# EnricoMiccoli/nodal

Hardware: AMD Instinct MI355X
Metric: circuits_per_sec (higher is better)
Workload: dtype f64; 1 GPU; cfg3: grid(1000) 1e6 nodes, sparse CSR path; n=999999, nnz=4995995, parallelism=one GPU

## Files before the change

nodal_amd/csrc/sagg.hip:

```cpp
#include <hip/hip_ext.h>

#include <atomic>
#include <type_traits>

#include "group.h"

int grounded_flags(nodal_ctx *h, uint8_t *flags_dev);

namespace {

using grp::TB;
constexpr int PW = 4;
constexpr int ACAP = 64;
constexpr int RCAP = 96;
constexpr int RCAP_SMALL = 512;
constexpr int RCAP_SMALL_ROWS = 16384;
inline int rcap_for(int64_t nc) { return nc <= RCAP_SMALL_ROWS ? RCAP_SMALL : RCAP; }
constexpr int W0_MAX = 32;
constexpr int COARSEST = 64;
constexpr int MAX_LEVELS = 12;
constexpr int MIS_ROUNDS = 6;
constexpr int TAIL_MAX_N = 1024;
constexpr int TAIL_LEVELS = 6;
constexpr int TAIL_LDS_BUDGET = 150 * 1024;
// ... 94 lines not shown
    bool kcycle = true;
    bool kfrozen = false;
    int kslot = -1, kcount = 0, ksamples = 0;
    int klevels = 1;
    int nu[3] = {2, 1, 2};
    bool dense_coarsest = true;
    DevBuf tail_stamps, tail_image, apcol, apval, aplen, bstat;
    DevBuf tail_op;
    bool tail_dense = false;
    DevBuf mvec;
    hipEvent_t ev_copy = nullptr;
    hipStream_t aux = nullptr;
    hipEvent_t ev_fork = nullptr, ev_join = nullptr, ev_flags = nullptr;
    bool aux_pending = false;
    bool aux_tried = false;
    bool want_flags = false;
    int flags_levels = 0;
    DevBuf stats, coarse_inv, mis_t, mis_m, mis_flag, mis_id, agg1, keys, rstart, cursor, lists;
    TailDesc td;
    uint64_t *host_stats = nullptr;
    bool sym_valid = false;
    uint64_t sym_epoch = 0;
    int64_t sym_n = 0, sym_nnz = 0;
    bool sym_general = false, sym_check = false;
    int32_t sym_floating = 0;
    hipGraph_t it_graph = nullptr;
    hipGraphExec_t it_exec = nullptr;
    uint64_t it_key = 0;
    bool refreshed = false;
    int last_iters = 0;
    int hint_iters = 0;
    int64_t hint_n = 0, hint_nnz = 0;
    int mblock_iters = 0;
    int64_t mblock_n = 0;
    unsigned long long sym_stats[MAX_LEVELS * ST_COUNT] = {0};
    SLevel *level(int l) {
        while ((int)pool.size() <= l) pool.push_back(new SLevel());
        return pool[l];
    }
    void drop_graph() {
        if (it_exec) (void)hipGraphExecDestroy(it_exec);
        if (it_graph) (void)hipGraphDestroy(it_graph);
        it_exec = nullptr;
        it_graph = nullptr;
        it_key = 0;
    }
    ~SHierarchy() {
        drop_graph();
        if (ev_copy) (void)hipEventDestroy(ev_copy);
        if (ev_fork) (void)hipEventDestroy(ev_fork);
        if (ev_join) (void)hipEventDestroy(ev_join);
        if (ev_flags) (void)hipEventDestroy(ev_flags);
        if (aux) (void)hipStreamDestroy(aux);
        for (SLevel *l : pool) {
            DevBuf *b[] = {&l->acol, &l->aval, &l->alen, &l->dinv, &l->agg, &l->pcol, &l->pval, &l->rcol,
                           &l->rval, &l->rlen, &l->vec, &l->part, &l->gflag, &l->avalf, &l->pvalf, &l->rvalf, &l->adcol,
                           &l->wcol, &l->wval, &l->wlen};
            for (DevBuf *x : b) x->release();
            delete l;
        }
        tail_image.release();
        tail_op.release();
        mvec.release();
        tail_stamps.release();
        bstat.release();
        apcol.release();
        apval.release();
        aplen.release();
        DevBuf *b[] = {&stats, &coarse_inv, &mis_t, &mis_m, &mis_flag, &mis_id, &agg1, &keys, &rstart, &cursor, &lists};
        for (DevBuf *x : b) x->release();
        if (host_stats) (void)hipHostFree(host_stats);
    }
};


constexpr int BSTAT_MAX = 65536;
__global__ __launch_bounds__(1024) void reduce_bstat(int nblocks, const uint32_t *__restrict__ bstat,
                                                     unsigned long long *__restrict__ stats, int slot_max,
                                                     int slot_sum) {
    __shared__ unsigned int s_max;
    __shared__ unsigned long long s_sum;
    if (threadIdx.x == 0) { s_max = 0; s_sum = 0; }
    __syncthreads();
    unsigned int m = 0;
    unsigned long long t = 0;
    for (int i = threadIdx.x; i < nblocks; i += 1024) {
        m = max(m, bstat[i]);
        t += bstat[BSTAT_MAX + i];
// ... 41 lines not shown
    if (far) atomicOr(&s_bad, 2u);
    __syncthreads();
    if (threadIdx.x == 0) {
        bstat[blockIdx.x] = s_len;
        bstat[BSTAT_MAX + blockIdx.x] = s_graded;
        if (s_bad & 1u) atomicOr(&stats[ST_BADDIAG], 1ull);
        if (s_bad & 2u) stats[ST_FARCOL] = 1ull;
    }
}

__global__ __launch_bounds__(TB) void csr_to_ell(int64_t n, int64_t ld, const int32_t *__restrict__ indptr,
                                                 const int32_t *__restrict__ indices,
                                                 const double *__restrict__ data, int32_t *__restrict__ col,
                                                 double *__restrict__ val, float *__restrict__ valf,
                                                 int32_t *__restrict__ len, double *__restrict__ dinv, int32_t wpad,
                                                 int16_t *__restrict__ dcol) {
    for (int64_t i = (int64_t)xcd_block() * TB + threadIdx.x; i < n; i += (int64_t)gridDim.x * TB) {
        const int32_t e0 = indptr[i], e1 = indptr[i + 1];
        double d = 1.0;
        for (int32_t e = e0; e < e1; ++e) {
            const int32_t c = indices[e];
            const double v = data[e];
            col[(int64_t)(e - e0) * ld + i] = c;
            if (dcol) dcol[(int64_t)(e - e0) * ld + i] = (int16_t)(c - (int32_t)i);
            val[(int64_t)(e - e0) * ld + i] = v;
            valf[(int64_t)(e - e0) * ld + i] = (float)v;
            if (c == (int32_t)i) d = v;
        }
        for (int32_t s = e1 - e0; s < wpad; ++s) {
            col[(int64_t)s * ld + i] = (int32_t)i;
            if (dcol) dcol[(int64_t)s * ld + i] = 0;
            val[(int64_t)s * ld + i] = 0.0;
            valf[(int64_t)s * ld + i] = 0.0f;
        }
        len[i] = e1 - e0;
// ... 1200 lines not shown
    for (int i = 0; i < n; ++i) {
        long double y = 0.0L, a = 0.0L;
        for (int j = 0; j < n; ++j) {
            y += (long double)T[(size_t)i * n + j] * b[j];
            a += fabsl((long double)T[(size_t)i * n + j] * b[j]);
        }
        const double den = (double)a;
        const double q = fabs(yd[i] - yc[i]) / den, qp = (double)(fabsl((long double)yd[i] - y) / a);
        d = !(q <= d) ? q : d;
        dp = !(qp <= dp) ? qp : dp;
    }
    fprintf(stderr, "[sagg] tail check: n_t %d, dense operator against the cycle d = %.3e (product alone %.3e)\n", n, d, dp);
    return NODAL_OK;
}

int form_tail_op(nodal_ctx *h, SHierarchy *H) {
    static const bool on = !(getenv("NODAL_SA_TAIL_DENSE") && atoi(getenv("NODAL_SA_TAIL_DENSE")) == 0);
    H->tail_dense = false;
    if (!on || H->tail < 0) return NODAL_OK;
    const TailDesc &d = H->td;
    const int n = d.lv[0].n;
    static std::atomic<int> cus[64];
    const int dev = h->device >= 0 && h->device < 64 ? h->device : 0;
    int ncu = cus[dev].load(std::memory_order_acquire);
    if (ncu == 0) {
        NODAL_HIP_TRY(h, hipDeviceGetAttribute(&ncu, hipDeviceAttributeMultiprocessorCount, h->device >= 0 ? h->device : 0));
        if (ncu < 1) ncu = 1;
        cus[dev].store(ncu, std::memory_order_release);
    }
    NODAL_HIP_TRY(h, H->tail_op.reserve((size_t)n * n * 8 + 64));
    const unsigned gr = (unsigned)(n < ncu ? n : ncu);
    double *T = H->tail_op.as<double>();
    const char *img = H->tail_image.as<char>();
    if (d.slots <= 8) k_tail_pack_op<8><<<gr, 1024, (size_t)d.lds_bytes, h->stream>>>(d, img, T);
// ... 68 lines not shown
                    "(worst row against its own bound: %.3e)\n", l, (long long)n, (int)L->wslots, (int)L->maxlen, dm, qm);
    return NODAL_OK;
}
int fold_self_check(nodal_ctx *h, SHierarchy *H) {
    static const bool check = getenv("NODAL_TRACE") && getenv("NODAL_SA_FOLD_CHECK") && atoi(getenv("NODAL_SA_FOLD_CHECK")) != 0;
    if (!check) return NODAL_OK;
    for (int l = 0; l + 1 < H->nlev; ++l) {
        if (!H->pool[l]->fold) continue;
        const bool last = l + 1 == H->tail || l + 1 == H->nlev - 1;
        if (last) NODAL_TRY(fold_check_level<double>(h, H, l, false));
        else NODAL_TRY(fold_check_level<cyc_t>(h, H, l, true));
    }
    return NODAL_OK;
}

int build_tail(nodal_ctx *h, SHierarchy *H, const unsigned long long *hs) {
    H->tail = -1;
    H->tail_dense = false;
    const int last = H->nlev - 1;
    auto up16 = [](int x) { return (x + 15) & ~15; };
    for (int t = 1; t <= last; ++t) {
        if (H->pool[t]->n > TAIL_MAX_N || last - t + 1 > TAIL_LEVELS) continue;
        TailDesc d;
        memset(&d, 0, sizeof d);
        d.nlev = last - t + 1;
        d.nu = getenv("NODAL_SA_TAIL_NU") ? atoi(getenv("NODAL_SA_TAIL_NU")) : 3;
        if (d.nu < 1) d.nu = 1;
        int off = 0;
        for (int k = 0; k < d.nlev; ++k) {
            const SLevel *L = H->pool[t + k];
// ... 39 lines not shown
        d.slots = d.nlev > 1 ? (d.lv[0].width + d.lv[0].lpr - 1) / d.lv[0].lpr : 1;
        if (d.slots > 32) continue;
        {
            static std::atomic<bool> lds_allowed[64][3];
            const int dev = h->device >= 0 && h->device < 64 ? h->device : 0;
            const int which = d.slots <= 8 ? 0 : (d.slots <= 16 ? 1 : 2);
            if (!lds_allowed[dev][which].load(std::memory_order_acquire)) {
                NODAL_HIP_TRY(h, hipFuncSetAttribute(tail_kernel(d.slots), hipFuncAttributeMaxDynamicSharedMemorySize,
                                                     TAIL_LDS_BUDGET));
                NODAL_HIP_TRY(h, hipFuncSetAttribute(tail_op_kernel(d.slots), hipFuncAttributeMaxDynamicSharedMemorySize,
                                                     TAIL_LDS_BUDGET));
                lds_allowed[dev][which].store(true, std::memory_order_release);
            }
        }
        NODAL_HIP_TRY(h, H->tail_image.reserve((size_t)d.image_bytes + 256));
        k_tail_pack<<<1, 1024, 0, h->stream>>>(d, H->tail_image.as<char>());
        NODAL_HIP_TRY(h, hipGetLastError());
        H->td = d;
        H->tail = t;
        NODAL_TRY(form_tail_op(h, H));
        break;
    }
    return NODAL_OK;
}

int sagg_refresh(nodal_ctx *h, SHierarchy *H, const int32_t *indptr0, const int32_t *indices0, const double *data0,
                 bool general, bool *ok) {
    *ok = false;
    hipStream_t st = h->stream;
    unsigned long long *dstats = H->stats.as<unsigned long long>();
    unsigned long long *hs = reinterpret_cast<unsigned long long *>(H->host_stats);
    NODAL_HIP_TRY(h, hipMemsetAsync(dstats, 0, (size_t)MAX_LEVELS * ST_COUNT * 8, st));
    SLevel *L0 = H->pool[0];
    const int64_t n0 = L0->n;
    {
        const unsigned gr = grid_for(n0);
        static const double spread = getenv("NODAL_SA_SPREAD") ? atof(getenv("NODAL_SA_SPREAD")) : 16.0;
        static const double share = getenv("NODAL_SA_SHARE") ? atof(getenv("NODAL_SA_SHARE")) : 0.9;
        row_stats<<<gr, TB, 0, st>>>(n0, indptr0, indices0, data0, share, spread, general, dstats, H->bstat.as<uint32_t>());
        reduce_bstat<<<1, 1024, 0, st>>>((int)gr, H->bstat.as<uint32_t>(), dstats, ST_MAXLEN, ST_GRADED);
    }
    csr_to_ell<<<grid_for(n0), TB, 0, st>>>(n0, L0->ld, indptr0, indices0, data0, L0->acol.as<int32_t>(),
                                           L0->aval.as<double>(), L0->avalf.as<float>(),
                                           L0->alen.as<int32_t>(), L0->dinv.as<double>(), L0->wfix,
                                           L0->d16 ? L0->adcol.as<int16_t>() : nullptr);
    NODAL_HIP_TRY(h, hipGetLastError());
    for (int l = 0; l + 1 < H->nlev; ++l) {
        SLevel *L = H->pool[l], *C = H->pool[l + 1];
        Ell A = L->A();
        A.width = L->maxlen;
        build_P<<<grid_for(L->n), TB, 0, st>>>(A, L->dinv.as<double>(), L->agg.as<int32_t>(), L->pcol.as<int32_t>(),
                                              L->pval.as<double>(), L->pvalf.as<float>(), omega_p(l));
        const bool forked = H->aux != nullptr && nodal_extra_streams_ok(h) &&
                            !(getenv("NODAL_SA_FORK") && atoi(getenv("NODAL_SA_FORK")) == 0);
        hipStream_t rst = st;
        if (forked) {
            NODAL_HIP_TRY(h, hipEventRecord(H->ev_fork, st));
            NODAL_HIP_TRY(h, hipStreamWaitEvent(H->aux, H->ev_fork, 0));
            H->aux_pending = true;
            NODAL_TRY(galerkin_product<true>(h, H, l, nullptr, 1));
// ... 21 lines not shown
        if (hs[(size_t)k * ST_COUNT + ST_BADDIAG] || hs[(size_t)k * ST_COUNT + ST_OVERFLOW]) return NODAL_OK;
    decide_folds(H, hs, false);
    NODAL_TRY(fold_self_check(h, H));
    *ok = true;
    return NODAL_OK;
}

}

void sagg_destroy(nodal_ctx *h) {
    delete static_cast<SHierarchy *>(h->sagg);
    h->sagg = nullptr;
}

static int sagg_setup_csr_body(nodal_ctx *h, int64_t n0, int64_t nnz0, const int32_t *indptr0, const int32_t *indices0,
                               const double *data0, bool general, bool check_floating, bool *accepted, int32_t *floating);

int sagg_setup_csr(nodal_ctx *h, int64_t n0, int64_t nnz0, const int32_t *indptr0, const int32_t *indices0,
                   const double *data0, bool general, bool check_floating, bool *accepted, int32_t *floating) {
    const int s = sagg_setup_csr_body(h, n0, nnz0, indptr0, indices0, data0, general, check_floating, accepted, floating);
    SHierarchy *H = static_cast<SHierarchy *>(h->sagg);
    if (H && H->aux && H->aux_pending && H->ev_flags) {
        if (hipEventRecord(H->ev_flags, H->aux) == hipSuccess) (void)hipStreamWaitEvent(h->stream, H->ev_flags, 0);
        H->aux_pending = false;
        (void)hipGetLastError();
    }
    return s;
}

static int sagg_setup_csr_body(nodal_ctx *h, int64_t n0, int64_t nnz0, const int32_t *indptr0, const int32_t *indices0,
                               const double *data0, bool general, bool check_floating, bool *accepted, int32_t *floating) {
    *accepted = false;
    *floating = 0;
    static const bool enabled = !(getenv("NODAL_SAGG") && atoi(getenv("NODAL_SAGG")) == 0);
    static const bool trace = getenv("NODAL_TRACE") != nullptr;
    if (!enabled) return NODAL_OK;
    SHierarchy *H = hierarchy_of(h);
    H->ready = false;
    hipStream_t st = h->stream;
    if (n0 >= (1ll << 30)) return NODAL_OK;
    static const bool reuse = !(getenv("NODAL_SA_REUSE") && atoi(getenv("NODAL_SA_REUSE")) == 0);
    if (reuse && H->sym_valid && H->sym_epoch == h->struct_epoch && H->sym_n == n0 && H->sym_nnz == nnz0 &&
        H->sym_general == general && H->sym_check == check_floating) {
        bool ok = false;
        NODAL_TRY(sagg_refresh(h, H, indptr0, indices0, data0, general, &ok));
        if (ok) {
            *floating = H->sym_floating;
            H->refreshed = true;
            H->ready = true;
            *accepted = true;
            if (trace) fprintf(stderr, "[sagg] symbolic setup kept (struct epoch %llu): values refreshed\n",
                               (unsigned long long)h->struct_epoch);
            return NODAL_OK;
        }
        if (trace) fprintf(stderr, "[sagg] the kept hierarchy does not take the new values: full setup\n");
    }
    H->sym_valid = false;
    H->refreshed = false;
    H->want_flags = check_floating;
    H->flags_levels = 0;
    H->last_iters = 0;
    H->drop_graph();
    NODAL_HIP_TRY(h, H->stats.reserve((size_t)MAX_LEVELS * ST_COUNT * 8 + 64));
    if (!H->host_stats)
        NODAL_HIP_TRY(h, hipHostMalloc(reinterpret_cast<void **>(&H->host_stats), (size_t)MAX_LEVELS * ST_COUNT * 8 + 64));
    unsigned long long *dstats = H->stats.as<unsigned long long>();
    unsigned long long *hs = reinterpret_cast<unsigned long long *>(H->host_stats);
    NODAL_HIP_TRY(h, hipMemsetAsync(dstats, 0, (size_t)MAX_LEVELS * ST_COUNT * 8, st));
    NODAL_HIP_TRY(h, H->bstat.reserve((size_t)2 * BSTAT_MAX * 4 + 64));
    {
        const unsigned gr = grid_for(n0);
        static const double spread = getenv("NODAL_SA_SPREAD") ? atof(getenv("NODAL_SA_SPREAD")) : 16.0;
        static const double share = getenv("NODAL_SA_SHARE") ? atof(getenv("NODAL_SA_SHARE")) : 0.9;
        row_stats<<<gr, TB, 0, st>>>(n0, indptr0, indices0, data0, share, spread, general, dstats, H->bstat.as<uint32_t>());
        reduce_bstat<<<1, 1024, 0, st>>>((int)gr, H->bstat.as<uint32_t>(), dstats, ST_MAXLEN, ST_GRADED);
    }
    NODAL_HIP_TRY(h, hipGetLastError());
    NODAL_HIP_TRY(h, hipMemcpyAsync(hs, dstats, ST_COUNT * 8, hipMemcpyDeviceToHost, st));
    NODAL_WAIT_STREAM(h, st);
    const int64_t bar = n0 / 100 < 32 ? (n0 / 100 > 0 ? n0 / 100 : 1) : 32;
    if (hs[ST_MAXLEN] > (unsigned long long)W0_MAX || hs[ST_MAXLEN] == 0 || hs[ST_BADDIAG] ||
        (int64_t)hs[ST_GRADED] >= bar) {
        if (trace)
            fprintf(stderr, "[sagg] declined: longest row %llu, graded nodes %llu (bar %lld), M-matrix %s\n",
                    hs[ST_MAXLEN], hs[ST_GRADED], (long long)bar, hs[ST_BADDIAG] ? "no" : "yes");
        return NODAL_OK;
    }
    SLevel *L0 = H->level(0);
    L0->n = n0;
    L0->ld = pad64(n0);
    L0->maxlen = (int32_t)hs[ST_MAXLEN];
    L0->nnz = nnz0;
    L0->wfix = choose_wfix(L0->maxlen, n0, nnz0, 8);
    L0->width = L0->wfix ? L0->wfix : L0->maxlen;
    NODAL_HIP_TRY(h, L0->acol.reserve((size_t)L0->width * L0->ld * 4 + 64));
    NODAL_HIP_TRY(h, L0->aval.reserve((size_t)L0->width * L0->ld * 8 + 64));
    NODAL_HIP_TRY(h, L0->avalf.reserve((size_t)L0->width * L0->ld * 4 + 64));
    NODAL_HIP_TRY(h, L0->alen.reserve((size_t)L0->ld * 4 + 64));
    NODAL_HIP_TRY(h, L0->dinv.reserve((size_t)L0->ld * 8 + 64));
    static const bool d16_env = !(getenv("NODAL_SA_D16") && atoi(getenv("NODAL_SA_D16")) == 0);
    L0->d16 = d16_env && hs[ST_FARCOL] == 0;
    if (L0->d16) NODAL_HIP_TRY(h, L0->adcol.reserve((size_t)L0->width * L0->ld * 2 + 64));
    csr_to_ell<<<grid_for(n0), TB, 0, st>>>(n0, L0->ld, indptr0, indices0, data0, L0->acol.as<int32_t>(),
                                           L0->aval.as<double>(), L0->avalf.as<float>(),
                                           L0->alen.as<int32_t>(), L0->dinv.as<double>(), L0->wfix,
                                           L0->d16 ? L0->adcol.as<int16_t>() : nullptr);
    NODAL_HIP_TRY(h, hipGetLastError());

    int l = 0;
    bool diag_last = false;
    for (;; ++l) {
        SLevel *L = H->level(l);
        if (L->n <= COARSEST && l > 0) break;
        if (l + 1 >= MAX_LEVELS) {
            if (trace) fprintf(stderr, "[sagg] declined: more than %d levels\n", MAX_LEVELS);
            return NODAL_OK;
        }
        bool declined = false, stop = false;
        NODAL_TRY(build_level(h, H, l, hs, &declined, &stop));
        if (declined) {
            if (trace)
                fprintf(stderr, "[sagg] declined at level %d (%lld rows): does not coarsen / over a cap / not positive "
// ... 39 lines not shown
        if (k > 0) {
            H->pool[k]->maxlen = (int32_t)s[ST_MAXLEN];
            H->pool[k]->nnz = (int64_t)s[ST_NNZ];
            H->pool[k]->wfix = choose_wfix(H->pool[k]->maxlen, H->pool[k]->n, H->pool[k]->nnz, APAD);
        }
        if (s[ST_OVERFLOW] || (k > 0 && s[ST_BADDIAG]) || s[ST_UNASSIGNED]) {
            if (trace) fprintf(stderr, "[sagg] declined: level %d over a cap / not positive\n", k);
            return NODAL_OK;
        }
    }
    diag_last = last->maxlen <= 1;
    H->dense_coarsest = !diag_last;
    if (H->dense_coarsest) {
        if (last->n > COARSEST) return NODAL_OK;
        NODAL_HIP_TRY(h, H->coarse_inv.reserve((size_t)last->n * last->n * 8 + 64));
        coarsest_inverse<<<1, 256, 0, st>>>(last->A(), H->coarse_inv.as<double>(),
                                            dstats + (size_t)l * ST_COUNT);
        NODAL_HIP_TRY(h, hipGetLastError());
    }
    for (int k = 0; k < H->nlev; ++k) {
        SLevel *L = H->pool[k];
        NODAL_HIP_TRY(h, L->vec.reserve((size_t)V_COUNT * L->ld * 8 + 256));
        NODAL_HIP_TRY(h, L->part.reserve(5 * DOT_BLOCKS * 8 + 512));
    }
    NODAL_TRY(build_tail(h, H, hs));

    if (!check_floating) {
        NODAL_HIP_TRY(h, hipMemcpyAsync(hs, dstats, (size_t)MAX_LEVELS * ST_COUNT * 8, hipMemcpyDeviceToHost, st));
        NODAL_WAIT_STREAM(h, st);
        if (hs[(size_t)l * ST_COUNT + ST_BADDIAG] & 2ull) return NODAL_OK;
    } else {
        uint32_t *fl = reinterpret_cast<uint32_t *>(dstats + (size_t)(MAX_LEVELS - 1) * ST_COUNT + ST_COUNT - 1);
        if (H->dense_coarsest) last_level_floating<<<1, 64, 0, st>>>(last->A(), last->gflag.as<uint8_t>(), fl);
        else any_unflagged<<<grid_for(last->n), TB, 0, st>>>(last->n, last->gflag.as<uint8_t>(), fl);
        NODAL_HIP_TRY(h, hipGetLastError());
        NODAL_HIP_TRY(h, hipMemcpyAsync(hs, dstats, (size_t)MAX_LEVELS * ST_COUNT * 8, hipMemcpyDeviceToHost, st));
        NODAL_WAIT_STREAM(h, st);
        if (hs[(size_t)l * ST_COUNT + ST_BADDIAG] & 2ull) {
            if (trace) fprintf(stderr, "[sagg] declined: coarsest matrix not positive definite\n");
            return NODAL_OK;
        }
        *floating = hs[(size_t)(MAX_LEVELS - 1) * ST_COUNT + ST_COUNT - 1] != 0 ? 1 : 0;
    }
    if (trace) {
        fprintf(stderr, "[sagg] levels (rows/entries/longest row/padded width):");
        for (int k = 0; k < H->nlev; ++k)
            fprintf(stderr, " %lld/%lld/%d/%d", (long long)H->pool[k]->n, (long long)H->pool[k]->nnz,
                    H->pool[k]->maxlen, H->pool[k]->wfix);
        fprintf(stderr, "  tail %d (%d register slots)  coarsest %s\n", H->tail, H->tail >= 0 ? H->td.slots : 0,
                H->dense_coarsest ? "dense" : "diagonal");
    }
    decide_folds(H, hs, trace);
    NODAL_TRY(fold_self_check(h, H));
    H->ready = true;
    *accepted = true;
    H->sym_valid = true;
    H->sym_epoch = h->struct_epoch;
    H->sym_n = n0;
    H->sym_nnz = nnz0;
    H->sym_general = general;
    H->sym_check = check_floating;
    H->sym_floating = *floating;
    memcpy(H->sym_stats, hs, sizeof H->sym_stats);
    return NODAL_OK;
}

int sagg_setup(nodal_ctx *h, bool *accepted, int32_t *floating) {
    return sagg_setup_csr(h, h->n, h->nnz, h->indptr.as<int32_t>(), h->indices.as<int32_t>(), h->data.as<double>(),
                          false, true, accepted, floating);
}

namespace {

int last_level(nodal_ctx *h, SHierarchy *H, int l, const double *b, double *out) {
    hipStream_t st = h->stream;
    SLevel *L = H->pool[l];
    const int64_t n = L->n;
    if (l == H->tail) return H->tail_dense ? tail_apply<1>(h, H, b, out) : tail_walk(h, H, b, out, 1);
    k_coarsest<<<grid_for(n), TB, 0, st>>>(n, H->dense_coarsest ? H->coarse_inv.as<double>() : nullptr,
                                           L->dinv.as<double>(), b, out);
    NODAL_HIP_TRY(h, hipGetLastError());
    return NODAL_OK;
}

void kcycle_schedule(SHierarchy *H, int it) {
    static const bool on = !(getenv("NODAL_SA_KFREEZE") && atoi(getenv("NODAL_SA_KFREEZE")) == 0);
    H->kfrozen = false;
    H->kslot = -1;
    if (!on || it < 0) return;
    if (it == 0) H->ksamples = 0;
    const bool adaptive = it < 4 || (it & 3) == 0;
    if (!adaptive && H->ksamples > 0) {
// ... 189 lines not shown
    hipStream_t st = h->stream;
    SHierarchy *H = hierarchy_of(h);
    if (do_setup) {
        bool accepted = false;
        int32_t floating = 0;
        NODAL_TRY(sagg_setup(h, &accepted, &floating));
        if (!accepted) return SAGG_DECLINED;
        if (floating) {
            *info = 1;
            *iters = 0;
            *resid = 0.0;
            return -2;
        }
    }
    if (!H->ready || H->pool[0]->n != n) return SAGG_DECLINED;
    h->amg_levels = H->nlev;
    static const int kc = getenv("NODAL_SA_KCYCLE") ? atoi(getenv("NODAL_SA_KCYCLE")) : 1;
    H->kcycle = kc != 0;
    H->klevels = getenv("NODAL_SA_KLEVELS") ? atoi(getenv("NODAL_SA_KLEVELS")) : 1;
    if (const char *e = getenv("NODAL_SA_NU")) {
        for (int k = 0; k < 3 && e[k] >= '1' && e[k] <= '3'; ++k) H->nu[k] = e[k] - '0';
    }

    const size_t vec = align_up((size_t)n * 8);
    NODAL_HIP_TRY(h, h->solver.reserve(6 * vec + 4 * MAX_PARTIALS * 8 + F_COUNT * 8 + 256));
    char *base = h->solver.as<char>();
    SolveBufs sb;
    sb.r = reinterpret_cast<double *>(base);
    sb.z = reinterpret_cast<cyc_t *>(base + vec);
    sb.p = reinterpret_cast<double *>(base + 2 * vec);
// ... 4 lines not shown
    sb.part_zap = sb.part_rz + MAX_PARTIALS;
    sb.part_rr = sb.part_zap + MAX_PARTIALS;
    sb.part_pap = sb.part_rr + MAX_PARTIALS;
    sb.sc = sb.part_pap + MAX_PARTIALS;
    sb.g0 = (int)grid_for(n, MAX_PARTIALS);
    double *x = h->x.as<double>();
    const Ell A0 = H->pool[0]->A();

    const double tol = 1e-13;
    f_set_scalars<<<1, 1, 0, st>>>(sb.sc, tol * tol);
    const double *dinv0 = H->pool[0]->dinv.as<double>();
    f_init<<<sb.g0, TB, 0, st>>>(b, x, sb.r, sb.Ap, dinv0, sb.x0, sb.part_rr, n);
    NODAL_HIP_TRY(h, hipGetLastError());

    const int64_t maxit = getenv("NODAL_FCG_MAXIT") ? atoll(getenv("NODAL_FCG_MAXIT")) : 2000;
    hipEvent_t e0 = h->ev[2], e1 = h->ev[3];
    h->kern_ms = 0;
    h->kern_launches = 0;
    double hs[F_COUNT];
    int64_t enqueued = 0;
    int batch = 6;
    if (H->last_iters > 6 && (H->refreshed || !do_setup)) batch = H->last_iters + 1 > 32 ? 32 : H->last_iters + 1;
    else if (H->hint_iters > 8 && H->hint_n == n && H->hint_nnz == H->pool[0]->nnz) {
        batch = (3 * H->hint_iters) / 4;
        if (batch > 32) batch = 32;
    }
    int status = 0;
    const bool poll_partials = !(getenv("NODAL_FCG_HOST_SUM") && atoi(getenv("NODAL_FCG_HOST_SUM")) == 0);
    double rr_prev = -1.0;
    int64_t it_prev = 0;
    int polls = 0;
    static const bool fuse_dir_env = !(getenv("NODAL_SA_FUSE_DIR") && atoi(getenv("NODAL_SA_FUSE_DIR")) == 0);
    const bool fuse_dir = fuse_dir_env && LPR_RAGGED == 1;
    static const bool graphs_env = getenv("NODAL_SA_GRAPH") && atoi(getenv("NODAL_SA_GRAPH")) != 0;
    auto iteration = [&](int it, bool timed) -> int {
        kcycle_schedule(H, graphs_env ? -1 : it);
        struct KReset {
            SHierarchy *H;
            ~KReset() { H->kfrozen = false; H->kslot = -1; }
        } kreset{H};
// ... 59 lines not shown
                if (cs == NODAL_OK && ce == hipSuccess && g && hipGraphInstantiate(&ex, g, nullptr, nullptr, 0) == hipSuccess) {
                    H->it_graph = g;
                    H->it_exec = ex;
                    H->it_key = key;
                } else {
                    if (g) (void)hipGraphDestroy(g);
                    (void)hipGetLastError();
                }
            } else {
                (void)hipGetLastError();
            }
        }
    } else if (H->it_exec && do_setup) {
        H->drop_graph();
    }
    while (status == 0) {
        for (int c = 0; c < batch;) {
            if (H->it_exec && c > 0 && c + 1 < batch && (enqueued & 1) == 0) {
                NODAL_HIP_TRY(h, hipGraphLaunch(H->it_exec, st));
                c += 2;
                enqueued += 2;
            } else {
                NODAL_TRY(iteration((int)enqueued, c == 0));
                ++c;
                ++enqueued;
            }
        }
        double rr_now = -1.0;
        {
            const size_t bytes = (size_t)(2 * MAX_PARTIALS + F_COUNT) * 8;
            double *stage = poll_partials ? static_cast<double *>(nodal_pinned_arena(h, bytes)) : nullptr;
            if (stage) {
                NODAL_HIP_TRY(h, hipMemcpyAsync(stage, sb.part_rr, bytes, hipMemcpyDeviceToHost, st));
                NODAL_WAIT_STREAM(h, st);
                memcpy(hs, stage + 2 * MAX_PARTIALS, F_COUNT * 8);
                double acc = 0.0;
                for (int k = 0; k < sb.g0; ++k) acc += stage[k];
                rr_now = acc;
            } else {
                NODAL_TRY(nodal_read_words(h, hs, sb.sc, F_COUNT * 8));
            }
        }
        ++polls;
        bool conv = hs[F_CONV + ((enqueued - 1) & 1)] != 0.0;
        bool host_conv = false;
        if (!conv && rr_now >= 0.0 && hs[F_FLAG] == 0.0 && hs[F_BB] > 0.0 && rr_now <= tol * tol * hs[F_BB]) {
            host_conv = true;
            hs[F_RR] = rr_now;
            hs[F_ITERS] = (double)enqueued;
        } else if (!conv && rr_now >= 0.0) {
            hs[F_RR] = rr_now;
        }
        float ms = 0;
        if (!(conv && !host_conv && hs[F_ITERS] <= (double)(enqueued - batch)) && hipEventElapsedTime(&ms, e0, e1) == hipSuccess) {
            h->kern_ms += ms;
            h->kern_launches += 1;
        }
        if (hs[F_FLAG] != 0.0 || !(hs[F_RR] == hs[F_RR])) status = 2;
        else if (conv || host_conv) status = 1;
        else if (enqueued >= maxit) status = 3;
        else {
            int next = 2;
            const double target = tol * tol * hs[F_BB];
            const double rr_ref = rr_prev > 0.0 ? rr_prev : hs[F_BB];
            const int64_t it_ref = rr_prev > 0.0 ? it_prev : 0;
            if (hs[F_RR] > 0.0 && hs[F_RR] < rr_ref && enqueued > it_ref) {
                const double rate = log(hs[F_RR] / rr_ref) / (double)(enqueued - it_ref);
                static const double look = getenv("NODAL_FCG_LOOK") ? atof(getenv("NODAL_FCG_LOOK")) : 0.75;
                next = (int)floor(look * log(target / hs[F_RR]) / rate);
            }
            if (next > enqueued) next = (int)enqueued;
            batch = next < 1 ? 1 : (next > 32 ? 32 : next);
            rr_prev = hs[F_RR];
            it_prev = enqueued;
        }
    }
    const int64_t its = status == 1 ? (int64_t)hs[F_ITERS] : enqueued;
    *iters = (int32_t)its;
    *resid = hs[F_BB] > 0 ? sqrt(hs[F_RR] / hs[F_BB]) : 0.0;
    const SLevel *L0 = H->pool[0];
    h->kern_alg = 12.0 * (double)L0->nnz + 4.0 * (double)n + 16.0 * (double)n;
    if (fuse_dir) h->kern_alg += 12.0 * (double)n;
    if (trace)
        fprintf(stderr, "[sagg] %d iterations (%lld enqueued, %d polls), relative residual %.2e, status %d\n", *iters,
                (long long)enqueued, polls, *resid, status);
    if (trace && H->tail >= 0 && H->td.stamps && !H->tail_dense) {
        long long ts[64];
        if (hipMemcpy(ts, H->td.stamps, sizeof ts, hipMemcpyDeviceToHost) == hipSuccess) {
            fprintf(stderr, "[sagg] tail phases (us):");
            for (int k = 1; k < (int)ts[63] && k < 63; ++k) fprintf(stderr, " %.2f", (double)(ts[k] - ts[k - 1]) * 0.01);
            fprintf(stderr, "  total %.2f, image %d B, lds %d B\n", (double)(ts[ts[63] - 1] - ts[0]) * 0.01,
                    H->td.image_bytes, H->td.lds_bytes);
// ... 19 lines not shown
```

Before: 163.7 circuits/s.

## Overlap SA-AMG setup host syncs with device work and enqueue solver iterations ahead

Removes several host stalls in the smoothed-aggregation setup and FCG solve. The level-0 ELL conversion is launched speculatively from a cached row-length hint before the stats readback completes, and is redone only if the hint fails. The coarsest inverse, tail packing and floating check can be forked onto an auxiliary stream, with the verdict read later during the solve. While the host polls the residual partials, the solver enqueues one extra iteration to keep the GPU busy. This adds considerable control complexity and rollback paths, and on convergence an ahead iteration is wasted.

```diff
diff --git a/nodal_amd/csrc/sagg.hip b/nodal_amd/csrc/sagg.hip
--- a/nodal_amd/csrc/sagg.hip
+++ b/nodal_amd/csrc/sagg.hip
@@ -132,6 +132,12 @@
     hipEvent_t ev_fork = nullptr, ev_join = nullptr, ev_flags = nullptr;
     bool aux_pending = false;
     bool aux_tried = false;
+    bool verdict_pending = false;
+    hipEvent_t verdict_ev = nullptr;
+    hipStream_t verdict_st = nullptr;
+    bool tail_join = false;
+    int verdict_level = 0;
+    hipEvent_t ev_time[2] = {nullptr, nullptr};
     bool want_flags = false;
     int flags_levels = 0;
     DevBuf stats, coarse_inv, mis_t, mis_m, mis_flag, mis_id, agg1, keys, rstart, cursor, lists;
@@ -149,6 +155,10 @@
     int last_iters = 0;
     int hint_iters = 0;
     int64_t hint_n = 0, hint_nnz = 0;
+    bool lay_valid = false;
+    int64_t lay_n = 0, lay_nnz = 0;
+    int32_t lay_maxlen = 0;
+    bool lay_far = false;
     int mblock_iters = 0;
     int64_t mblock_n = 0;
     unsigned long long sym_stats[MAX_LEVELS * ST_COUNT] = {0};
@@ -169,6 +179,8 @@
         if (ev_fork) (void)hipEventDestroy(ev_fork);
         if (ev_join) (void)hipEventDestroy(ev_join);
         if (ev_flags) (void)hipEventDestroy(ev_flags);
+        for (hipEvent_t e : ev_time)
+            if (e) (void)hipEventDestroy(e);
         if (aux) (void)hipStreamDestroy(aux);
         for (SLevel *l : pool) {
             DevBuf *b[] = {&l->acol, &l->aval, &l->alen, &l->dinv, &l->agg, &l->pcol, &l->pval, &l->rcol,
@@ -190,6 +202,11 @@
         if (host_stats) (void)hipHostFree(host_stats);
     }
 };
+
+bool sagg_eager() {
+    static const bool on = !(getenv("NODAL_SA_EAGER") && atoi(getenv("NODAL_SA_EAGER")) == 0);
+    return on;
+}
 
 
 constexpr int BSTAT_MAX = 65536;
@@ -261,11 +278,12 @@
                                                  const double *__restrict__ data, int32_t *__restrict__ col,
                                                  double *__restrict__ val, float *__restrict__ valf,
                                                  int32_t *__restrict__ len, double *__restrict__ dinv, int32_t wpad,
-                                                 int16_t *__restrict__ dcol) {
+                                                 int16_t *__restrict__ dcol, int32_t width) {
     for (int64_t i = (int64_t)xcd_block() * TB + threadIdx.x; i < n; i += (int64_t)gridDim.x * TB) {
         const int32_t e0 = indptr[i], e1 = indptr[i + 1];
+        const int32_t ec = e1 - e0 > width ? e0 + width : e1;
         double d = 1.0;
-        for (int32_t e = e0; e < e1; ++e) {
+        for (int32_t e = e0; e < ec; ++e) {
             const int32_t c = indices[e];
             const double v = data[e];
             col[(int64_t)(e - e0) * ld + i] = c;
@@ -1496,10 +1514,14 @@
     return NODAL_OK;
 }
 
+bool tail_dense_wanted() {
+    static const bool on = !(getenv("NODAL_SA_TAIL_DENSE") && atoi(getenv("NODAL_SA_TAIL_DENSE")) == 0);
+    return on;
+}
+
 int form_tail_op(nodal_ctx *h, SHierarchy *H) {
-    static const bool on = !(getenv("NODAL_SA_TAIL_DENSE") && atoi(getenv("NODAL_SA_TAIL_DENSE")) == 0);
     H->tail_dense = false;
-    if (!on || H->tail < 0) return NODAL_OK;
+    if (!tail_dense_wanted() || H->tail < 0) return NODAL_OK;
     const TailDesc &d = H->td;
     const int n = d.lv[0].n;
     static std::atomic<int> cus[64];
@@ -1598,6 +1620,13 @@
     return NODAL_OK;
 }
 
+int tail_pack(nodal_ctx *h, SHierarchy *H) {
+    if (H->tail < 0) return NODAL_OK;
+    k_tail_pack<<<1, 1024, 0, h->stream>>>(H->td, H->tail_image.as<char>());
+    NODAL_HIP_TRY(h, hipGetLastError());
+    return form_tail_op(h, H);
+}
+
 int build_tail(nodal_ctx *h, SHierarchy *H, const unsigned long long *hs) {
     H->tail = -1;
     H->tail_dense = false;
@@ -1667,14 +1696,22 @@
             }
         }
         NODAL_HIP_TRY(h, H->tail_image.reserve((size_t)d.image_bytes + 256));
-        k_tail_pack<<<1, 1024, 0, h->stream>>>(d, H->tail_image.as<char>());
-        NODAL_HIP_TRY(h, hipGetLastError());
+        if (tail_dense_wanted()) NODAL_HIP_TRY(h, H->tail_op.reserve((size_t)d.lv[0].n * d.lv[0].n * 8 + 64));
         H->td = d;
         H->tail = t;
-        NODAL_TRY(form_tail_op(h, H));
         break;
     }
     return NODAL_OK;
+}
+
+void read_verdict(SHierarchy *H, bool trace, bool *declined, int32_t *floating) {
+    const unsigned long long *hv = reinterpret_cast<const unsigned long long *>(H->host_stats) + (size_t)MAX_LEVELS * ST_COUNT;
+    *declined = (hv[(size_t)H->verdict_level * ST_COUNT + ST_BADDIAG] & 2ull) != 0;
+    if (*declined) {
+        if (trace) fprintf(stderr, "[sagg] declined: coarsest matrix not positive definite\n");
+        return;
+    }
+    *floating = hv[(size_t)(MAX_LEVELS - 1) * ST_COUNT + ST_COUNT - 1] != 0 ? 1 : 0;
 }
 
 int sagg_refresh(nodal_ctx *h, SHierarchy *H, const int32_t *indptr0, const int32_t *indices0, const double *data0,
@@ -1696,7 +1733,7 @@
     csr_to_ell<<<grid_for(n0), TB, 0, st>>>(n0, L0->ld, indptr0, indices0, data0, L0->acol.as<int32_t>(),
                                            L0->aval.as<double>(), L0->avalf.as<float>(),
                                            L0->alen.as<int32_t>(), L0->dinv.as<double>(), L0->wfix,
-                                           L0->d16 ? L0->adcol.as<int16_t>() : nullptr);
+                                           L0->d16 ? L0->adcol.as<int16_t>() : nullptr, L0->width);
     NODAL_HIP_TRY(h, hipGetLastError());
     for (int l = 0; l + 1 < H->nlev; ++l) {
         SLevel *L = H->pool[l], *C = H->pool[l + 1];
@@ -1748,11 +1785,14 @@
 }
 
 static int sagg_setup_csr_body(nodal_ctx *h, int64_t n0, int64_t nnz0, const int32_t *indptr0, const int32_t *indices0,
-                               const double *data0, bool general, bool check_floating, bool *accepted, int32_t *floating);
-
-int sagg_setup_csr(nodal_ctx *h, int64_t n0, int64_t nnz0, const int32_t *indptr0, const int32_t *indices0,
-                   const double *data0, bool general, bool check_floating, bool *accepted, int32_t *floating) {
-    const int s = sagg_setup_csr_body(h, n0, nnz0, indptr0, indices0, data0, general, check_floating, accepted, floating);
+                               const double *data0, bool general, bool check_floating, bool *accepted, int32_t *floating,
+                               bool defer_verdict);
+
+static int sagg_setup_joined(nodal_ctx *h, int64_t n0, int64_t nnz0, const int32_t *indptr0, const int32_t *indices0,
+                             const double *data0, bool general, bool check_floating, bool *accepted, int32_t *floating,
+                             bool defer_verdict) {
+    const int s = sagg_setup_csr_body(h, n0, nnz0, indptr0, indices0, data0, general, check_floating, accepted, floating,
+                                      defer_verdict);
     SHierarchy *H = static_cast<SHierarchy *>(h->sagg);
     if (H && H->aux && H->aux_pending && H->ev_flags) {
         if (hipEventRecord(H->ev_flags, H->aux) == hipSuccess) (void)hipStreamWaitEvent(h->stream, H->ev_flags, 0);
@@ -1762,8 +1802,14 @@
     return s;
 }
 
+int sagg_setup_csr(nodal_ctx *h, int64_t n0, int64_t nnz0, const int32_t *indptr0, const int32_t *indices0,
+                   const double *data0, bool general, bool check_floating, bool *accepted, int32_t *floating) {
+    return sagg_setup_joined(h, n0, nnz0, indptr0, indices0, data0, general, check_floating, accepted, floating, false);
+}
+
 static int sagg_setup_csr_body(nodal_ctx *h, int64_t n0, int64_t nnz0, const int32_t *indptr0, const int32_t *indices0,
-                               const double *data0, bool general, bool check_floating, bool *accepted, int32_t *floating) {
+                               const double *data0, bool general, bool check_floating, bool *accepted, int32_t *floating,
+                               bool defer_verdict) {
     *accepted = false;
     *floating = 0;
     static const bool enabled = !(getenv("NODAL_SAGG") && atoi(getenv("NODAL_SAGG")) == 0);
@@ -1772,6 +1818,10 @@
     SHierarchy *H = hierarchy_of(h);
     H->ready = false;
     hipStream_t st = h->stream;
+    if (H->verdict_pending) {
+        if (H->tail_join) (void)hipStreamWaitEvent(st, H->ev_join, 0);
+        H->verdict_pending = H->tail_join = false;
+    }
     if (n0 >= (1ll << 30)) return NODAL_OK;
     static const bool reuse = !(getenv("NODAL_SA_REUSE") && atoi(getenv("NODAL_SA_REUSE")) == 0);
     if (reuse && H->sym_valid && H->sym_epoch == h->struct_epoch && H->sym_n == n0 && H->sym_nnz == nnz0 &&
@@ -1797,7 +1847,7 @@
     H->drop_graph();
     NODAL_HIP_TRY(h, H->stats.reserve((size_t)MAX_LEVELS * ST_COUNT * 8 + 64));
     if (!H->host_stats)
-        NODAL_HIP_TRY(h, hipHostMalloc(reinterpret_cast<void **>(&H->host_stats), (size_t)MAX_LEVELS * ST_COUNT * 8 + 64));
+        NODAL_HIP_TRY(h, hipHostMalloc(reinterpret_cast<void **>(&H->host_stats), (size_t)2 * MAX_LEVELS * ST_COUNT * 8 + 64));
     unsigned long long *dstats = H->stats.as<unsigned long long>();
     unsigned long long *hs = reinterpret_cast<unsigned long long *>(H->host_stats);
     NODAL_HIP_TRY(h, hipMemsetAsync(dstats, 0, (size_t)MAX_LEVELS * ST_COUNT * 8, st));
@@ -1811,35 +1861,62 @@
     }
     NODAL_HIP_TRY(h, hipGetLastError());
     NODAL_HIP_TRY(h, hipMemcpyAsync(hs, dstats, ST_COUNT * 8, hipMemcpyDeviceToHost, st));
-    NODAL_WAIT_STREAM(h, st);
+    static const bool d16_env = !(getenv("NODAL_SA_D16") && atoi(getenv("NODAL_SA_D16")) == 0);
+    SLevel *L0 = H->level(0);
+    auto layout0 = [&](int32_t maxlen, bool far) -> int {
+        L0->n = n0;
+        L0->ld = pad64(n0);
+        L0->maxlen = maxlen;
+        L0->nnz = nnz0;
+        L0->wfix = choose_wfix(L0->maxlen, n0, nnz0, 8);
+        L0->width = L0->wfix ? L0->wfix : L0->maxlen;
+        NODAL_HIP_TRY(h, L0->acol.reserve((size_t)L0->width * L0->ld * 4 + 64));
+        NODAL_HIP_TRY(h, L0->aval.reserve((size_t)L0->width * L0->ld * 8 + 64));
+        NODAL_HIP_TRY(h, L0->avalf.reserve((size_t)L0->width * L0->ld * 4 + 64));
+        NODAL_HIP_TRY(h, L0->alen.reserve((size_t)L0->ld * 4 + 64));
+        NODAL_HIP_TRY(h, L0->dinv.reserve((size_t)L0->ld * 8 + 64));
+        L0->d16 = d16_env && !far;
+        if (L0->d16) NODAL_HIP_TRY(h, L0->adcol.reserve((size_t)L0->width * L0->ld * 2 + 64));
+        csr_to_ell<<<grid_for(n0), TB, 0, st>>>(n0, L0->ld, indptr0, indices0, data0, L0->acol.as<int32_t>(),
+                                               L0->aval.as<double>(), L0->avalf.as<float>(),
+                                               L0->alen.as<int32_t>(), L0->dinv.as<double>(), L0->wfix,
+                                               L0->d16 ? L0->adcol.as<int16_t>() : nullptr, L0->width);
+        NODAL_HIP_TRY(h, hipGetLastError());
+        return NODAL_OK;
+    };
+    const bool hinted = sagg_eager() && H->lay_valid && H->lay_n == n0 && H->lay_nnz == nnz0 && H->lay_maxlen > 0 &&
+                        H->lay_maxlen <= W0_MAX;
+    if (hinted) {
+        if (!H->ev_copy) NODAL_HIP_TRY(h, hipEventCreateWithFlags(&H->ev_copy, hipEventDisableTiming));
+        NODAL_HIP_TRY(h, hipEventRecord(H->ev_copy, st));
+        NODAL_TRY(layout0(H->lay_maxlen, H->lay_far));
+        NODAL_WAIT_EVENT(h, H->ev_copy, st);
+    } else {
+        NODAL_WAIT_STREAM(h, st);
+    }
+    H->lay_valid = false;
     const int64_t bar = n0 / 100 < 32 ? (n0 / 100 > 0 ? n0 / 100 : 1) : 32;
-    if (hs[ST_MAXLEN] > (unsigned long long)W0_MAX || hs[ST_MAXLEN] == 0 || hs[ST_BADDIAG] ||
-        (int64_t)hs[ST_GRADED] >= bar) {
+    const bool declined0 = hs[ST_MAXLEN] > (unsigned long long)W0_MAX || hs[ST_MAXLEN] == 0 || hs[ST_BADDIAG] ||
+                           (int64_t)hs[ST_GRADED] >= bar;
+    const bool held = hinted && !declined0 && hs[ST_MAXLEN] == (unsigned long long)H->lay_maxlen &&
+                      (hs[ST_FARCOL] != 0) == H->lay_far;
+    if (hinted && !held && trace)
+        fprintf(stderr, "[sagg] level-0 hint (longest row %d, far columns %d) does not hold for this matrix (longest row "
+                        "%llu, far columns %d%s): restart on the true values\n",
+                (int)H->lay_maxlen, (int)H->lay_far, hs[ST_MAXLEN], (int)(hs[ST_FARCOL] != 0),
+                declined0 ? ", declined" : "");
+    if (declined0) {
         if (trace)
             fprintf(stderr, "[sagg] declined: longest row %llu, graded nodes %llu (bar %lld), M-matrix %s\n",
                     hs[ST_MAXLEN], hs[ST_GRADED], (long long)bar, hs[ST_BADDIAG] ? "no" : "yes");
         return NODAL_OK;
     }
-    SLevel *L0 = H->level(0);
-    L0->n = n0;
-    L0->ld = pad64(n0);
-    L0->maxlen = (int32_t)hs[ST_MAXLEN];
-    L0->nnz = nnz0;
-    L0->wfix = choose_wfix(L0->maxlen, n0, nnz0, 8);
-    L0->width = L0->wfix ? L0->wfix : L0->maxlen;
-    NODAL_HIP_TRY(h, L0->acol.reserve((size_t)L0->width * L0->ld * 4 + 64));
-    NODAL_HIP_TRY(h, L0->aval.reserve((size_t)L0->width * L0->ld * 8 + 64));
-    NODAL_HIP_TRY(h, L0->avalf.reserve((size_t)L0->width * L0->ld * 4 + 64));
-    NODAL_HIP_TRY(h, L0->alen.reserve((size_t)L0->ld * 4 + 64));
-    NODAL_HIP_TRY(h, L0->dinv.reserve((size_t)L0->ld * 8 + 64));
-    static const bool d16_env = !(getenv("NODAL_SA_D16") && atoi(getenv("NODAL_SA_D16")) == 0);
-    L0->d16 = d16_env && hs[ST_FARCOL] == 0;
-    if (L0->d16) NODAL_HIP_TRY(h, L0->adcol.reserve((size_t)L0->width * L0->ld * 2 + 64));
-    csr_to_ell<<<grid_for(n0), TB, 0, st>>>(n0, L0->ld, indptr0, indices0, data0, L0->acol.as<int32_t>(),
-                                           L0->aval.as<double>(), L0->avalf.as<float>(),
-                                           L0->alen.as<int32_t>(), L0->dinv.as<double>(), L0->wfix,
-                                           L0->d16 ? L0->adcol.as<int16_t>() : nullptr);
-    NODAL_HIP_TRY(h, hipGetLastError());
+    if (!held) NODAL_TRY(layout0((int32_t)hs[ST_MAXLEN], hs[ST_FARCOL] != 0));
+    H->lay_valid = true;
+    H->lay_n = n0;
+    H->lay_nnz = nnz0;
+    H->lay_maxlen = (int32_t)hs[ST_MAXLEN];
+    H->lay_far = hs[ST_FARCOL] != 0;
 
     int l = 0;
     bool diag_last = false;
@@ -1909,33 +1986,66 @@
     if (H->dense_coarsest) {
         if (last->n > COARSEST) return NODAL_OK;
         NODAL_HIP_TRY(h, H->coarse_inv.reserve((size_t)last->n * last->n * 8 + 64));
-        coarsest_inverse<<<1, 256, 0, st>>>(last->A(), H->coarse_inv.as<double>(),
-                                            dstats + (size_t)l * ST_COUNT);
-        NODAL_HIP_TRY(h, hipGetLastError());
     }
     for (int k = 0; k < H->nlev; ++k) {
         SLevel *L = H->pool[k];
         NODAL_HIP_TRY(h, L->vec.reserve((size_t)V_COUNT * L->ld * 8 + 256));
         NODAL_HIP_TRY(h, L->part.reserve(5 * DOT_BLOCKS * 8 + 512));
     }
+    static const bool self_checks = getenv("NODAL_TRACE") && (getenv("NODAL_SA_TAIL_CHECK") || getenv("NODAL_SA_FOLD_CHECK"));
+    const bool defer = defer_verdict && check_floating && sagg_eager() && !self_checks;
+    static const bool fork_allowed = !(getenv("NODAL_SA_FORK") && atoi(getenv("NODAL_SA_FORK")) == 0);
+    const bool forked = defer && fork_allowed && H->aux != nullptr && H->ev_fork && H->ev_join && nodal_extra_streams_ok(h);
     NODAL_TRY(build_tail(h, H, hs));
-
+    hipStream_t main_st = h->stream;
+    struct StreamGuard {
+        nodal_ctx *h;
+        hipStream_t keep;
+        ~StreamGuard() { h->stream = keep; }
+    } guard{h, main_st};
+    if (forked) {
+        NODAL_HIP_TRY(h, hipEventRecord(H->ev_fork, main_st));
+        NODAL_HIP_TRY(h, hipStreamWaitEvent(H->aux, H->ev_fork, 0));
+        H->aux_pending = true;
+        h->stream = H->aux;
+        st = H->aux;
+    }
+    if (H->dense_coarsest) {
+        coarsest_inverse<<<1, 256, 0, st>>>(last->A(), H->coarse_inv.as<double>(),
+                                            dstats + (size_t)l * ST_COUNT);
+        NODAL_HIP_TRY(h, hipGetLastError());
+    }
+    NODAL_TRY(tail_pack(h, H));
+
+    unsigned long long *hv = hs + (size_t)MAX_LEVELS * ST_COUNT;
     if (!check_floating) {
-        NODAL_HIP_TRY(h, hipMemcpyAsync(hs, dstats, (size_t)MAX_LEVELS * ST_COUNT * 8, hipMemcpyDeviceToHost, st));
+        NODAL_HIP_TRY(h, hipMemcpyAsync(hv, dstats, (size_t)MAX_LEVELS * ST_COUNT * 8, hipMemcpyDeviceToHost, st));
         NODAL_WAIT_STREAM(h, st);
-        if (hs[(size_t)l * ST_COUNT + ST_BADDIAG] & 2ull) return NODAL_OK;
+        if (hv[(size_t)l * ST_COUNT + ST_BADDIAG] & 2ull) return NODAL_OK;
     } else {
         uint32_t *fl = reinterpret_cast<uint32_t *>(dstats + (size_t)(MAX_LEVELS - 1) * ST_COUNT + ST_COUNT - 1);
         if (H->dense_coarsest) last_level_floating<<<1, 64, 0, st>>>(last->A(), last->gflag.as<uint8_t>(), fl);
         else any_unflagged<<<grid_for(last->n), TB, 0, st>>>(last->n, last->gflag.as<uint8_t>(), fl);
         NODAL_HIP_TRY(h, hipGetLastError());
-        NODAL_HIP_TRY(h, hipMemcpyAsync(hs, dstats, (size_t)MAX_LEVELS * ST_COUNT * 8, hipMemcpyDeviceToHost, st));
-        NODAL_WAIT_STREAM(h, st);
-        if (hs[(size_t)l * ST_COUNT + ST_BADDIAG] & 2ull) {
-            if (trace) fprintf(stderr, "[sagg] declined: coarsest matrix not positive definite\n");
-            return NODAL_OK;
-        }
-        *floating = hs[(size_t)(MAX_LEVELS - 1) * ST_COUNT + ST_COUNT - 1] != 0 ? 1 : 0;
+        NODAL_HIP_TRY(h, hipMemcpyAsync(hv, dstats, (size_t)MAX_LEVELS * ST_COUNT * 8, hipMemcpyDeviceToHost, st));
+        H->verdict_level = l;
+        if (defer) {
+            H->verdict_ev = forked ? H->ev_join : H->ev_copy;
+            H->verdict_st = st;
+            NODAL_HIP_TRY(h, hipEventRecord(H->verdict_ev, st));
+            H->verdict_pending = true;
+            H->tail_join = forked;
+            if (forked) {
+                H->aux_pending = false;
+                h->stream = main_st;
+                st = main_st;
+            }
+        } else {
+            NODAL_WAIT_STREAM(h, st);
+            bool declined = false;
+            read_verdict(H, trace, &declined, floating);
+            if (declined) return NODAL_OK;
+        }
     }
     if (trace) {
         fprintf(stderr, "[sagg] levels (rows/entries/longest row/padded width):");
@@ -1957,12 +2067,13 @@
     H->sym_check = check_floating;
     H->sym_floating = *floating;
     memcpy(H->sym_stats, hs, sizeof H->sym_stats);
+    if (!H->verdict_pending) memcpy(H->sym_stats, hs + (size_t)MAX_LEVELS * ST_COUNT, sizeof H->sym_stats);
     return NODAL_OK;
 }
 
 int sagg_setup(nodal_ctx *h, bool *accepted, int32_t *floating) {
-    return sagg_setup_csr(h, h->n, h->nnz, h->indptr.as<int32_t>(), h->indices.as<int32_t>(), h->data.as<double>(),
-                          false, true, accepted, floating);
+    return sagg_setup_joined(h, h->n, h->nnz, h->indptr.as<int32_t>(), h->indices.as<int32_t>(), h->data.as<double>(),
+                             false, true, accepted, floating, true);
 }
 
 namespace {
@@ -1971,6 +2082,10 @@
     hipStream_t st = h->stream;
     SLevel *L = H->pool[l];
     const int64_t n = L->n;
+    if (H->tail_join) {
+        NODAL_HIP_TRY(h, hipStreamWaitEvent(st, H->ev_join, 0));
+        H->tail_join = false;
+    }
     if (l == H->tail) return H->tail_dense ? tail_apply<1>(h, H, b, out) : tail_walk(h, H, b, out, 1);
     k_coarsest<<<grid_for(n), TB, 0, st>>>(n, H->dense_coarsest ? H->coarse_inv.as<double>() : nullptr,
                                            L->dinv.as<double>(), b, out);
@@ -2190,6 +2305,9 @@
         }
     }
     if (!H->ready || H->pool[0]->n != n) return SAGG_DECLINED;
+    const int levels_before = h->amg_levels;
+    const double kern_ms_before = h->kern_ms;
+    const int64_t kern_launches_before = h->kern_launches;
     h->amg_levels = H->nlev;
     static const int kc = getenv("NODAL_SA_KCYCLE") ? atoi(getenv("NODAL_SA_KCYCLE")) : 1;
     H->kcycle = kc != 0;
@@ -2224,16 +2342,25 @@
     NODAL_HIP_TRY(h, hipGetLastError());
 
     const int64_t maxit = getenv("NODAL_FCG_MAXIT") ? atoll(getenv("NODAL_FCG_MAXIT")) : 2000;
-    hipEvent_t e0 = h->ev[2], e1 = h->ev[3];
+    const bool eager = sagg_eager();
+    if (eager) {
+        for (hipEvent_t &e : H->ev_time)
+            if (!e) NODAL_HIP_TRY(h, hipEventCreate(&e));
+        if (!H->ev_copy) NODAL_HIP_TRY(h, hipEventCreateWithFlags(&H->ev_copy, hipEventDisableTiming));
+    }
+    hipEvent_t tpair[2][2] = {{h->ev[2], h->ev[3]}, {eager ? H->ev_time[0] : h->ev[2], eager ? H->ev_time[1] : h->ev[3]}};
+    hipEvent_t e0 = tpair[0][0], e1 = tpair[0][1];
     h->kern_ms = 0;
     h->kern_launches = 0;
     double hs[F_COUNT];
     int64_t enqueued = 0;
     int batch = 6;
+    double more = 0.0;
     if (H->last_iters > 6 && (H->refreshed || !do_setup)) batch = H->last_iters + 1 > 32 ? 32 : H->last_iters + 1;
     else if (H->hint_iters > 8 && H->hint_n == n && H->hint_nnz == H->pool[0]->nnz) {
         batch = (3 * H->hint_iters) / 4;
         if (batch > 32) batch = 32;
+        more = (double)(H->hint_iters - batch);
     }
     int status = 0;
     const bool poll_partials = !(getenv("NODAL_FCG_HOST_SUM") && atoi(getenv("NODAL_FCG_HOST_SUM")) == 0);
@@ -2323,25 +2450,67 @@
     } else if (H->it_exec && do_setup) {
         H->drop_graph();
     }
+    int64_t seen = 0;
+    int bi = 0;
+    bool ahead = false;
     while (status == 0) {
-        for (int c = 0; c < batch;) {
+        for (int c = ahead ? 1 : 0; c < batch;) {
             if (H->it_exec && c > 0 && c + 1 < batch && (enqueued & 1) == 0) {
                 NODAL_HIP_TRY(h, hipGraphLaunch(H->it_exec, st));
                 c += 2;
                 enqueued += 2;
             } else {
+                if (c == 0) { e0 = tpair[bi & 1][0]; e1 = tpair[bi & 1][1]; }
                 NODAL_TRY(iteration((int)enqueued, c == 0));
                 ++c;
                 ++enqueued;
             }
         }
+        if (H->verdict_pending) {
+            if (H->tail_join) NODAL_HIP_TRY(h, hipStreamWaitEvent(st, H->ev_join, 0));
+            H->tail_join = false;
+            H->verdict_pending = false;
+            NODAL_WAIT_EVENT(h, H->verdict_ev, H->verdict_st);
+            bool declined = false;
+            int32_t floating = 0;
+            read_verdict(H, trace, &declined, &floating);
+            memcpy(H->sym_stats, reinterpret_cast<const unsigned long long *>(H->host_stats) + (size_t)MAX_LEVELS * ST_COUNT,
+                   sizeof H->sym_stats);
+            H->sym_floating = floating;
+            if (declined || floating) {
+                h->amg_levels = levels_before;
+                h->kern_ms = kern_ms_before;
+                h->kern_launches = kern_launches_before;
+                if (declined) {
+                    H->ready = false;
+                    H->sym_valid = false;
+                    return SAGG_DECLINED;
+                }
+                *info = 1;
+                *iters = 0;
+                *resid = 0.0;
+                return -2;
+            }
+        }
+        seen = enqueued;
+        ahead = false;
         double rr_now = -1.0;
         {
             const size_t bytes = (size_t)(2 * MAX_PARTIALS + F_COUNT) * 8;
             double *stage = poll_partials ? static_cast<double *>(nodal_pinned_arena(h, bytes)) : nullptr;
             if (stage) {
                 NODAL_HIP_TRY(h, hipMemcpyAsync(stage, sb.part_rr, bytes, hipMemcpyDeviceToHost, st));
-                NODAL_WAIT_STREAM(h, st);
+                if (eager && more >= 2.0 && seen < maxit) {
+                    NODAL_HIP_TRY(h, hipEventRecord(H->ev_copy, st));
+                    e0 = tpair[(bi + 1) & 1][0];
+                    e1 = tpair[(bi + 1) & 1][1];
+                    NODAL_TRY(iteration((int)enqueued, true));
+                    ++enqueued;
+                    ahead = true;
+                    NODAL_WAIT_EVENT(h, H->ev_copy, st);
+                } else {
+                    NODAL_WAIT_STREAM(h, st);
+                }
                 memcpy(hs, stage + 2 * MAX_PARTIALS, F_COUNT * 8);
                 double acc = 0.0;
                 for (int k = 0; k < sb.g0; ++k) acc += stage[k];
@@ -2351,40 +2520,46 @@
             }
         }
         ++polls;
-        bool conv = hs[F_CONV + ((enqueued - 1) & 1)] != 0.0;
+        bool conv = hs[F_CONV + ((seen - 1) & 1)] != 0.0;
         bool host_conv = false;
         if (!conv && rr_now >= 0.0 && hs[F_FLAG] == 0.0 && hs[F_BB] > 0.0 && rr_now <= tol * tol * hs[F_BB]) {
             host_conv = true;
             hs[F_RR] = rr_now;
-            hs[F_ITERS] = (double)enqueued;
+            hs[F_ITERS] = (double)seen;
         } else if (!conv && rr_now >= 0.0) {
             hs[F_RR] = rr_now;
         }
         float ms = 0;
-        if (!(conv && !host_conv && hs[F_ITERS] <= (double)(enqueued - batch)) && hipEventElapsedTime(&ms, e0, e1) == hipSuccess) {
+        if (!(conv && !host_conv && hs[F_ITERS] <= (double)(seen - batch)) &&
+            hipEventElapsedTime(&ms, tpair[bi & 1][0], tpair[bi & 1][1]) == hipSuccess) {
             h->kern_ms += ms;
             h->kern_launches += 1;
         }
+        ++bi;
         if (hs[F_FLAG] != 0.0 || !(hs[F_RR] == hs[F_RR])) status = 2;
         else if (conv || host_conv) status = 1;
-        else if (enqueued >= maxit) status = 3;
+        else if (seen >= maxit) status = 3;
         else {
             int next = 2;
+            double est = 0.0;
             const double target = tol * tol * hs[F_BB];
             const double rr_ref = rr_prev > 0.0 ? rr_prev : hs[F_BB];
             const int64_t it_ref = rr_prev > 0.0 ? it_prev : 0;
-            if (hs[F_RR] > 0.0 && hs[F_RR] < rr_ref && enqueued > it_ref) {
-                const double rate = log(hs[F_RR] / rr_ref) / (double)(enqueued - it_ref);
+            if (hs[F_RR] > 0.0 && hs[F_RR] < rr_ref && seen > it_ref) {
+                const double rate = log(hs[F_RR] / rr_ref) / (double)(seen - it_ref);
                 static const double look = getenv("NODAL_FCG_LOOK") ? atof(getenv("NODAL_FCG_LOOK")) : 0.75;
                 next = (int)floor(look * log(target / hs[F_RR]) / rate);
-            }
-            if (next > enqueued) next = (int)enqueued;
+                est = log(target / hs[F_RR]) / rate;
+            }
+            if (next > seen) next = (int)seen;
             batch = next < 1 ? 1 : (next > 32 ? 32 : next);
+            more = est - (double)batch;
             rr_prev = hs[F_RR];
-            it_prev = enqueued;
-        }
-    }
-    const int64_t its = status == 1 ? (int64_t)hs[F_ITERS] : enqueued;
+            it_prev = seen;
+        }
+    }
+    if (ahead) NODAL_WAIT_STREAM(h, st);
+    const int64_t its = status == 1 ? (int64_t)hs[F_ITERS] : seen;
     *iters = (int32_t)its;
     *resid = hs[F_BB] > 0 ? sqrt(hs[F_RR] / hs[F_BB]) : 0.0;
     const SLevel *L0 = H->pool[0];
```

New measurement: 166.3 circuits/s (median of 5 runs). No clear change (+1.5%).
